# joybio/multiPrime

Measured on AMD Instinct MI355X. Metric: candidate x sequence coverage evals/s, higher is better.
Workload: dtype u32; 1 GPU; synthetic MSA 1048576 x 1000, k=18, v=1, 8 candidates/window, 950 windows, strict -c 2,3,-1 per GPU x 1 GPU(s) = BASELINE configs[3] itself (SURVEY 8d input 4; synthetic 1M x 1 kb; shape 1x1: row shards x window groups); rows_per_gpu=1048576, rows_total=1048576, cols=1000, k=18, variation=1, candidates_per_window=8, windows=950, parallelism=one GPU holds every row

## Files before the change

multiprime_amd/csrc/common.hpp:

```cpp
#pragma once

#include "../../include/mprime.h"

#include <hip/hip_runtime.h>

#include <algorithm>
#include <cstdarg>
#include <cstdio>
#include <cstdlib>
#include <cstring>
#include <numeric>
#include <utility>
#include <chrono>
#include <mutex>
#include <unordered_map>
#include <vector>

namespace mp {

constexpr int kBlock = 256;
constexpr uint32_t kEmpty = 0xFFFFFFFFu;
constexpr int kHashSlots = 4096;
constexpr int kHashLimit = 3584;
constexpr int kEvalCC = 8;
// ... 13 lines not shown

template <int NQ> struct NibT {
    uint64_t q[NQ];
    __device__ void clear() {
#pragma unroll
        for (int i = 0; i < NQ; i++) q[i] = 0;
    }
    __device__ uint32_t get(int j) const {
        const int wi = j >> 4;
        uint64_t w = q[0];
#pragma unroll
        for (int i = 1; i < NQ; i++) w = wi == i ? q[i] : w;
        return (uint32_t)(w >> (4 * (j & 15))) & 15u;
    }
    __device__ void set(int j, uint32_t v) {
        const int wi = j >> 4, sh = 4 * (j & 15);
#pragma unroll
        for (int i = 0; i < NQ; i++)
            if (wi == i) q[i] = (q[i] & ~(15ull << sh)) | ((uint64_t)v << sh);
    }
    __device__ void shift_up(int n) {
        const int s = 4 * n, ws = s >> 6, bs = s & 63;
        if (s == 0) return;
        uint64_t out[NQ];
#pragma unroll
        for (int i = 0; i < NQ; i++) {
            uint64_t a = 0, b = 0;
#pragma unroll
            for (int t = 0; t < NQ; t++) {
                if (t == i - ws) a = q[t];
                if (t == i - ws - 1) b = q[t];
            }
            out[i] = bs ? (a << bs) | (b >> (64 - bs)) : a;
        }
#pragma unroll
        for (int i = 0; i < NQ; i++) q[i] = out[i];
    }
};
typedef NibT<2> Nib;

struct EvalForm {
    enum Path : int8_t { None, RowsNarrow, RowsWide, Bits, BitsX } path = None;
    int8_t bits_shape = 0;
    int8_t chain_shape = -1;
    bool use_prog = false;
    int8_t x_shape = 0;
    int8_t row_variant = 0;
    int8_t row_vmode = 0;
};

}

struct Lap {
    bool on = getenv("MP_TRACE") != nullptr;
    hipStream_t st;
    std::chrono::steady_clock::time_point t = std::chrono::steady_clock::now();
    explicit Lap(hipStream_t s) : st(s) {}
    void operator()(const char *what) {
        if (!on) return;
        (void)hipStreamSynchronize(st);
        auto now = std::chrono::steady_clock::now();
        fprintf(stderr, "[mprime] %-28s %8.3f ms\n", what, std::chrono::duration<double, std::milli>(now - t).count());
        t = now;
    }
};

#ifndef MP_HIST_CM64
#define MP_HIST_CM64 2
#endif

struct mp_ctx {
    char err[512] = {0};
    int dev = 0;
    hipStream_t stream = nullptr;
    const void *rot_block = nullptr;
    size_t rot_cleared = 0;
    hipStream_t alt_stream = nullptr;
    int64_t bytes = 0;
    int n_rows = 0, n_pad = 0, n_chunks = 0, max_len = 0, ustride = 0;
    int reserve_cols = 0;
    uint32_t *planes = nullptr, *cum = nullptr, *ung = nullptr;
    unsigned long long *cols = nullptr;
    int32_t *lead = nullptr, *rstrip = nullptr, *rlen = nullptr;
    int p0 = 0, n_win = 0, k = 0, v = 0;
    bool wide = false;
    unsigned long long *excl = nullptr;
    int32_t *patch_count = nullptr, *patch_off = nullptr, *patch_cursor = nullptr;
    uint32_t *patch_words = nullptr;
    int32_t *patch_rows = nullptr;
    int n_patch = 0, max_patch = 0;
    bool p64 = false;
    mp::ExRec *ex = nullptr;
    int ex_cap = 0;
    int *ex_count = nullptr, *err_flag = nullptr;
    std::vector<mp::ExRec> ex_host;
    std::vector<mp::ExRec> ex_raw;
    hipStream_t ex_stream = nullptr;
    int ex_pending = 0;
    std::mutex ex_mu;
    int32_t *extra_off = nullptr;
    uint32_t *extra_words = nullptr;
    int n_extra = 0;
    std::vector<int32_t> h_patch_off, h_extra_off;
    uint32_t *pplanes = nullptr, *pvalid = nullptr;
    uint32_t *qplanes = nullptr, *qvalid = nullptr;
    bool qp_dirty = true;
    mp::PatchWin *pwin = nullptr;
    size_t pp_words = 0, pv_words = 0;
    int max_npw = 0;
    bool pp_dirty = true;
    unsigned long long *g_key = nullptr;
    uint32_t *g_cnt = nullptr, *g_min = nullptr;
    uint32_t *g_gap = nullptr;
    int32_t *g_idx = nullptr;
    int g_slots = 0;
    long long u_cap = 0, u_n = 0;
    uint32_t *u_b0 = nullptr, *u_b1 = nullptr, *u_g = nullptr;
    int32_t *u_count = nullptr, *u_first = nullptr, *labels = nullptr, *u_over = nullptr, *u_wcount = nullptr;
    int64_t *u_wbase = nullptr;
    unsigned long long *u_total = nullptr;
    std::vector<int64_t> h_wbase;
    std::vector<int32_t> h_wcount;
    double gate_threshold = 0;
    std::vector<uint8_t> h_wskip;
    uint8_t *dm_loss = nullptr;
    double *dm_dg = nullptr;
    std::vector<uint8_t> dm_loss_host;
    std::vector<double> dm_dg_host;
    unsigned long long *mask_f = nullptr, *mask_r = nullptr;
    size_t mask_words = 0;
    int n_masks = 0;
    int n_cand = 0, n_items = 0, n_padded = 0;
    mp::EvalItem *items = nullptr;
    uint4 *cand_n = nullptr;
    uint32_t *cand_symT = nullptr, *cand_diff = nullptr, *chain_events = nullptr;
    mp::ChainItem *chain_items = nullptr;
    void *x_items = nullptr;
    uint32_t *x_events = nullptr;
    int32_t *x_cand_out = nullptr;
    int x_n = 0, x_n_events = 0;
    int32_t *table_ids = nullptr;
    int n_chain = 0, n_table = 0, n_events = 0, max_steps = 0;
    std::vector<mp::ChainItem> h_chains;
    std::vector<uint32_t> h_events;
    std::vector<int32_t> h_cand_out;
    uint32_t *chain_prog = nullptr;
    size_t chain_prog_n = 0;
    mp::EvalForm form;
    mp::SlideBand *slide_bands = nullptr;
    uint32_t *slide_iters = nullptr, *slide_recs = nullptr;
    size_t slide_n_iters = 0;
    int slide_items = 0, slide_n_bands = 0, slide_max_items = 0, slide_ns = 0, slide_gw = 0;
    uint32_t slide_spos = 0, slide_fmask = 0, slide_rmask = 0, slide_fpos = 0, slide_rpos = 0;
    bool slide_fast = false;
    mp::ChainItem *chain_rest = nullptr;
    mp::ChainItem *chain_slid = nullptr;
    int n_rest = 0, rest_max_steps = 0;
    unsigned launch_seq = 0;
    int32_t *cand_out = nullptr;
    uint64_t sF = 0, sR = 0;
    unsigned long long *tmp_out = nullptr;
    int tmp_out_n = 0;
    struct PoolBlock { void *p; size_t bytes; hipEvent_t released; };
    std::vector<hipEvent_t> pool_events;
    std::unordered_map<void *, size_t> pool_live;
    std::vector<PoolBlock> pool;
    size_t pool_bytes = 0;
    long long pool_hits = 0, pool_misses = 0;
    int pool_on = -1;
    std::mutex pool_mu;
    unsigned long long *stats_buf = nullptr;
    size_t stats_buf_n = 0;
    std::vector<std::pair<hipEvent_t, hipEvent_t>> ev_busy, ev_free;
    double ev_ms = 0;
    std::vector<float> ev_samples, ev_last;
    int ev_n = 0;
    uint8_t *h_stage = nullptr;
    size_t h_stage_bytes = 0;
    bool h_stage_pinned = false;
    uint8_t *h_stats = nullptr;
    size_t h_stats_bytes = 0, stats_pending_f = 0, stats_pending_t = 0;
    bool h_stats_pinned = false;
    hipEvent_t stats_ev = nullptr;
    uint8_t *h_ring = nullptr;
    bool h_ring_pinned = false;
    hipEvent_t h_ring_ev[3] = {nullptr, nullptr, nullptr};
    uint8_t *sq_bytes = nullptr;
    int64_t *sq_roff = nullptr;
    unsigned long long *sq_code = nullptr, *sq_flag = nullptr;
    int64_t *sq_woff = nullptr;
    int32_t sq_n = 0;
    size_t sq_total = 0, sq_words = 0;
    std::vector<int64_t> sq_roff_host;
    int32_t *ot_out = nullptr;
    int64_t ot_n = 0;
    std::vector<uint8_t> ot_key;
    double ot_ms[4] = {0, 0, 0, 0};
    int64_t ot_counts[7] = {0, 0, 0, 0, 0, 0, 0};
    std::vector<int32_t> otc_out;
    std::vector<uint8_t> otc_key;
    uint8_t *an_code = nullptr;
    uint32_t *an_kmer = nullptr;
    int32_t *an_table = nullptr;
    int32_t *an_col = nullptr, *an_colinv = nullptr;
    int32_t an_n = 0, an_L = 0, an_slots = 0;
    int32_t an_par[6] = {0, 0, 0, 0, 0, 0};
    double an_ms[5] = {0, 0, 0, 0, 0};
    int64_t an_counts[3] = {0, 0, 0};
    int32_t an_both = 0;
    uint8_t *cl_code = nullptr;
    int64_t *cl_off = nullptr;
    int32_t cl_n = 0;
    size_t cl_total = 0;
    std::vector<int64_t> cl_off_host;
    double cl_ms[5] = {0, 0, 0, 0, 0};
    int64_t cl_counts[3] = {0, 0, 0};
    bool cl_rev = false;
    uint32_t *ani_sk = nullptr;
    int32_t *ani_sizes = nullptr;
    uint32_t *ani_tab = nullptr;
    int32_t ani_n = 0, ani_s = 0;
    uint32_t *ani_or = nullptr;
    bool ani_strands = false;
    double ani_ms[2] = {0, 0};
    int64_t ani_counts[2] = {0, 0};
    uint8_t *st_bytes = nullptr;
    int64_t *st_off = nullptr;
    int32_t st_n = 0;
    size_t st_total = 0;
    std::vector<int64_t> st_off_host;
    uint8_t *st_parity = nullptr;
    int32_t st_an = 0, st_stride = 0, st_width = 0;
    int32_t *st_d0 = nullptr, *st_end = nullptr, *st_meta = nullptr, *st_wfin = nullptr;
    uint8_t *st_arow = nullptr;
    uint16_t *st_runlen = nullptr, *st_qstart = nullptr;
    int32_t *st_ins = nullptr, *st_acol = nullptr;
    int32_t *st_colmap = nullptr;
    uint8_t *st_rows = nullptr;
    int32_t *st_colcnt = nullptr;
    double st_ms[8] = {0, 0, 0, 0, 0, 0, 0, 0};
    int64_t st_counts[6] = {0, 0, 0, 0, 0, 0};
    mp::DegeState *dege = nullptr;
    uint64_t *ont_keys = nullptr;
    int32_t *ont_q = nullptr;
    int32_t ont_n = 0, ont_max_len = 0;
    double ont_ms = 0;
    int64_t ont_counts[2] = {0, 0};
    mp::SetScreen *ss = nullptr;
    double ss_ms[4] = {0, 0, 0, 0};
    int64_t ss_counts[8] = {0, 0, 0, 0, 0, 0, 0, 0};
    void *comm = nullptr;
    int n_ranks = 0, rank = 0;
    uint8_t *comm_scratch = nullptr;
    size_t comm_scratch_n = 0;
};

namespace mp {


inline size_t wsz(const mp_ctx *c) { return c->wide ? 2 : 1; }

inline int fail(mp_ctx *c, int code, const char *fmt, ...) {
    va_list ap;
    va_start(ap, fmt);
    vsnprintf(c->err, sizeof c->err, fmt, ap);
    va_end(ap);
    return code;
}

#define HIPCK(c, call)                                                                                   \
    do {                                                                                                 \
        hipError_t e_ = (call);                                                                          \
        if (e_ != hipSuccess) return fail((c), MP_ERR_DEVICE, "%s: %s", #call, hipGetErrorString(e_));  \
    } while (0)

void *pool_take(mp_ctx *c, size_t bytes);
bool pool_give(mp_ctx *c, void *p, size_t bytes);
void pool_drain(mp_ctx *c);
void pool_drain_all();
void pool_register(mp_ctx *c, bool alive);
void pool_note(mp_ctx *c, void *p, size_t bytes);
size_t pool_forget(mp_ctx *c, void *p, size_t claimed);

template <typename T>
int dev_alloc(mp_ctx *c, T **p, size_t n) {
    *p = nullptr;
    if (n == 0) n = 1;
    if (void *q = pool_take(c, n * sizeof(T))) {
        *p = (T *)q;
        pool_note(c, q, n * sizeof(T));
        c->bytes += (int64_t)(n * sizeof(T));
        return MP_OK;
    }
    hipError_t e = hipMalloc((void **)p, n * sizeof(T));
    if (e != hipSuccess) {
        (void)hipGetLastError();
        pool_drain_all();
        e = hipMalloc((void **)p, n * sizeof(T));
    }
    if (e != hipSuccess) return fail(c, MP_ERR_NOMEM, "hipMalloc(%zu bytes): %s", n * sizeof(T), hipGetErrorString(e));
    pool_note(c, (void *)*p, n * sizeof(T));
    c->bytes += (int64_t)(n * sizeof(T));
    return MP_OK;
}

template <typename T>
// ... 38 lines not shown
```

multiprime_amd/csrc/evalslide.hip:

```cpp
#include "common.hpp"
#include "bitslice.hpp"
#include "slidecore.hpp"
#include "evalslide.hpp"
#include "chainbody.hpp"

using namespace mp;

namespace {

typedef unsigned int u32x4 __attribute__((ext_vector_type(4)));
typedef unsigned int u32x2 __attribute__((ext_vector_type(2)));

struct SlideKernArgs {
    SlideArgs A;
    const uint32_t *cols32;
    const uint32_t *excl32;
    int nw32;
    unsigned long long *out;
    int wc, wc_pad;
    int max_items;
    int n_slide_blocks;
    EvalChainArgs chain;
    unsigned long long *clear;
    uint32_t n_clear;
    int patch_words;
    unsigned long long *stamps;
};

template <int GW>
struct DevEnv {
    const SlideKernArgs &K;
    __amdgpu_buffer_rsrc_t rs_cols, rs_excl;
    int voff, lane;
    uint32_t row_bytes;
    bool live;
    uint32_t *ring;
    uint32_t *tab;
    uint32_t itv;
    uint32_t live_mask;

    __device__ __forceinline__ DevEnv(const SlideKernArgs &k) : K(k) {}
    __device__ __forceinline__ void progress(int quarter) const {
#ifndef SLIDE_NO_PRIO
        if (quarter <= 0) __builtin_amdgcn_s_setprio(3);
        else if (quarter == 1) __builtin_amdgcn_s_setprio(2);
        else if (quarter == 2) __builtin_amdgcn_s_setprio(1);
        else __builtin_amdgcn_s_setprio(0);
#endif
    }
    __device__ __forceinline__ void stamp(int i) const {
        if (K.stamps && threadIdx.x == 0) K.stamps[(size_t)blockIdx.x * 8 + i] = wall_clock64();
    }
    __device__ __forceinline__ SlideBand uband(int b) const {
        const SlideBand *p = K.A.bands + b;
        SlideBand r;
        r.w0 = __builtin_amdgcn_readfirstlane(p->w0); r.n_win = __builtin_amdgcn_readfirstlane(p->n_win);
        r.item0 = __builtin_amdgcn_readfirstlane(p->item0); r.n_items = __builtin_amdgcn_readfirstlane(p->n_items);
        r.iter0 = __builtin_amdgcn_readfirstlane(p->iter0); r.pad = 0;
        return r;
    }
    __device__ __forceinline__ void load_iters(int idx) { itv = K.A.iters[(size_t)idx + (size_t)lane]; }
    __device__ __forceinline__ uint32_t iter_word(int j) const { return (uint32_t)__builtin_amdgcn_readlane((int)itv, j); }
    typedef const uint32_t __attribute__((address_space(4))) * ConstWords;
    struct Rec { uint32_t w[8], sm_lo, sm_hi, flags; ConstWords p; };
    __device__ __forceinline__ Rec load_rec(int item) const {
        Rec r;
        r.p = (ConstWords)(K.A.recs + (size_t)__builtin_amdgcn_readfirstlane(item) * kSlideRec);
#pragma unroll
        for (int q = 0; q < 8; q++) r.w[q] = r.p[q];
        r.sm_lo = r.p[24]; r.sm_hi = r.p[25]; r.flags = r.p[28];
        return r;
    }
    __device__ __forceinline__ uint32_t rec_word(const Rec &r, int q) const {
        return q < 8 ? r.w[q] : (q == 24 ? r.sm_lo : (q == 25 ? r.sm_hi : (q == 28 ? r.flags : r.p[q])));
    }
    __device__ __forceinline__ uint32_t rec_word_dyn(const Rec &r, int q) const { return r.p[q]; }
    template <int AUX = 0>
    __device__ __forceinline__ void load(__amdgpu_buffer_rsrc_t rs, int soff, uint32_t (&d)[GW]) const {
        if constexpr (GW == 4) {
            const u32x4 v = __builtin_amdgcn_raw_buffer_load_b128(rs, voff, soff, AUX);
            d[0] = v.x; d[1] = v.y; d[2] = v.z; d[3] = v.w;
        } else if constexpr (GW == 2) {
            const u32x2 v = __builtin_amdgcn_raw_buffer_load_b64(rs, voff, soff, AUX);
            d[0] = v.x; d[1] = v.y;
        } else {
            d[0] = __builtin_amdgcn_raw_buffer_load_b32(rs, voff, soff, AUX);
        }
    }
#ifndef SLIDE_EXP_ONE_ROW
#define SLIDE_EXP_ONE_ROW 0
#endif
#ifndef SLIDE_COL_AUX
#define SLIDE_COL_AUX 2
#endif
#ifndef SLIDE_EVT_AUX
#define SLIDE_EVT_AUX 0
#endif
    __device__ __forceinline__ void fetch(uint32_t row_off, uint32_t (&d)[GW]) const {
        load<SLIDE_COL_AUX>(rs_cols, SLIDE_EXP_ONE_ROW == 1 || SLIDE_EXP_ONE_ROW == 3 ? 0 : (int)row_off, d);
    }
    __device__ __forceinline__ void fetch_event(uint32_t row_off, uint32_t (&d)[GW]) const {
        load<SLIDE_EVT_AUX>(rs_cols, SLIDE_EXP_ONE_ROW == 1 || SLIDE_EXP_ONE_ROW == 2 ? 0 : (int)row_off, d);
    }
    __device__ __forceinline__ void valid_of(uint32_t row_off, uint32_t (&v)[GW]) const {
        load(rs_excl, (int)row_off, v);
#pragma unroll
        for (int i = 0; i < GW; i++) v[i] = bop<kSlAndNot>(live_mask, v[i], 0u);
    }
    __device__ __forceinline__ void ring_put(uint32_t *p, const uint32_t (&v)[GW]) const {
        if constexpr (GW == 4) *reinterpret_cast<u32x4 *>(p) = u32x4{v[0], v[1], v[2], v[3]};
        else if constexpr (GW == 2) *reinterpret_cast<u32x2 *>(p) = u32x2{v[0], v[1]};
        else p[0] = v[0];
    }
    __device__ __forceinline__ void ring_get(const uint32_t *p, uint32_t (&v)[GW]) const {
        if constexpr (GW == 4) { const u32x4 t = *reinterpret_cast<const u32x4 *>(p); v[0] = t.x; v[1] = t.y; v[2] = t.z; v[3] = t.w; }
        else if constexpr (GW == 2) { const u32x2 t = *reinterpret_cast<const u32x2 *>(p); v[0] = t.x; v[1] = t.y; }
        else v[0] = p[0];
    }
    __device__ __forceinline__ void ring_zero(int k) {
        uint32_t z[GW];
#pragma unroll
        for (int i = 0; i < GW; i++) z[i] = 0u;
        for (int s = 0; s < k; s++) ring_put(ring + s * (64 * GW), z);
    }
    __device__ __forceinline__ uint32_t ring_step() const { return 64u * GW * (uint32_t)sizeof(uint32_t); }
    __device__ __forceinline__ uint32_t *ring_at(uint32_t off) const { return reinterpret_cast<uint32_t *>(reinterpret_cast<char *>(ring) + off); }
    __device__ __forceinline__ void ring_write(uint32_t off, const uint32_t (&in)[GW]) { ring_put(ring_at(off), in); }
    __device__ __forceinline__ void ring_read(uint32_t off, uint32_t (&o)[GW]) const { ring_get(ring_at(off), o); }
    __device__ __forceinline__ void commit(int idx, const uint32_t (&accPF)[8], const uint32_t (&accR)[4]) {
        uint32_t x0 = accPF[0], x1 = accPF[1], x2 = accPF[2], x3 = accPF[3], x4 = accPF[4], x5 = accPF[5], x6 = accPF[6], x7 = accPF[7];
        uint32_t x8 = accR[0], x9 = accR[1], x10 = accR[2], x11 = accR[3];
        asm volatile(
            "s_nop 1\n\t"
            "v_add_u32_dpp %0, %0, %0 row_ror:4 row_mask:0xf bank_mask:0x5\n\t"
            "v_add_u32_dpp %2, %2, %2 row_ror:4 row_mask:0xf bank_mask:0x5\n\t"
            "v_add_u32_dpp %4, %4, %4 row_ror:4 row_mask:0xf bank_mask:0x5\n\t"
            "v_add_u32_dpp %6, %6, %6 row_ror:4 row_mask:0xf bank_mask:0x5\n\t"
            "v_add_u32_dpp %8, %8, %8 row_ror:4 row_mask:0xf bank_mask:0x5\n\t"
            "v_add_u32_dpp %10, %10, %10 row_ror:4 row_mask:0xf bank_mask:0x5\n\t"
            "v_add_u32_dpp %0, %1, %1 row_ror:4 row_mask:0xf bank_mask:0xa\n\t"
            "v_add_u32_dpp %2, %3, %3 row_ror:4 row_mask:0xf bank_mask:0xa\n\t"
            "v_add_u32_dpp %4, %5, %5 row_ror:4 row_mask:0xf bank_mask:0xa\n\t"
            "v_add_u32_dpp %6, %7, %7 row_ror:4 row_mask:0xf bank_mask:0xa\n\t"
            "v_add_u32_dpp %8, %9, %9 row_ror:4 row_mask:0xf bank_mask:0xa\n\t"
            "v_add_u32_dpp %10, %11, %11 row_ror:4 row_mask:0xf bank_mask:0xa\n\t"
            "v_add_u32_dpp %0, %0, %0 row_ror:8 row_mask:0xf bank_mask:0x3\n\t"
            "v_add_u32_dpp %4, %4, %4 row_ror:8 row_mask:0xf bank_mask:0x3\n\t"
            "v_add_u32_dpp %8, %8, %8 row_ror:8 row_mask:0xf bank_mask:0x3\n\t"
            "v_add_u32_dpp %0, %2, %2 row_ror:8 row_mask:0xf bank_mask:0xc\n\t"
            "v_add_u32_dpp %4, %6, %6 row_ror:8 row_mask:0xf bank_mask:0xc\n\t"
            "v_add_u32_dpp %8, %10, %10 row_ror:8 row_mask:0xf bank_mask:0xc\n\t"
            "v_add_u32_dpp %0, %0, %0 quad_perm:[1,0,3,2] row_mask:0xf bank_mask:0xf\n\t"
            "v_add_u32_dpp %4, %4, %4 quad_perm:[1,0,3,2] row_mask:0xf bank_mask:0xf\n\t"
            "v_add_u32_dpp %8, %8, %8 quad_perm:[1,0,3,2] row_mask:0xf bank_mask:0xf\n\t"
            "v_add_u32_dpp %0, %0, %0 quad_perm:[2,3,0,1] row_mask:0xf bank_mask:0xf\n\t"
            "v_add_u32_dpp %4, %4, %4 quad_perm:[2,3,0,1] row_mask:0xf bank_mask:0xf\n\t"
            "v_add_u32_dpp %8, %8, %8 quad_perm:[2,3,0,1] row_mask:0xf bank_mask:0xf\n\t"
            "s_nop 1"
            : "+v"(x0), "+v"(x1), "+v"(x2), "+v"(x3), "+v"(x4), "+v"(x5), "+v"(x6), "+v"(x7), "+v"(x8), "+v"(x9), "+v"(x10), "+v"(x11));
        typedef unsigned int u32pair __attribute__((ext_vector_type(2)));
        const u32pair s01 = __builtin_amdgcn_permlane16_swap(x0, x4, false, false);
        const uint32_t a = s01.x + s01.y;
        const u32pair s22 = __builtin_amdgcn_permlane16_swap(x8, x8, false, false);
        const uint32_t b = s22.x + s22.y;
        const u32pair h = __builtin_amdgcn_permlane32_swap(a, b, false, false);
        const uint32_t tot = h.x + h.y;
        if (lane < 48 && (lane & 3) == 0) atomicAdd(&tab[idx * 12 + (lane >> 4) * 4 + ((lane >> 2) & 3)], tot);
    }
};

#ifndef SLIDE_MIN_WAVES
#define SLIDE_MIN_WAVES 1
#endif
template <int LV, int GW, bool FAST>
__global__ __launch_bounds__(kBlock, GW == 4 ? 1 : SLIDE_MIN_WAVES) void eval_slide_kernel(const SlideKernArgs K) {
    extern __shared__ __align__(16) uint32_t lds[];
    clear_counters(K.clear, K.n_clear, blockIdx.x, gridDim.x);
    if (K.stamps && threadIdx.x == 0) K.stamps[(size_t)blockIdx.x * 8] = wall_clock64();
    if ((int)blockIdx.x >= K.n_slide_blocks) {
        const unsigned pb = blockIdx.x - (unsigned)K.n_slide_blocks, wv = threadIdx.x >> 6;
#ifndef SLIDE_PATCH_PRIO
#define SLIDE_PATCH_PRIO 3
#endif
        __builtin_amdgcn_s_setprio(SLIDE_PATCH_PRIO);
        if (K.patch_words == 1) {
            const bool negative = (int)pb >= K.chain.patch.n_blocks;
            const unsigned unit = (pb - (negative ? (unsigned)K.chain.patch.n_blocks : 0u)) * (kBlock / 64) + wv;
            eval_patch_wave<LV>(K.chain, lds + wv * 12, lds + 64 + wv * (64 * kPatchEvents), unit, negative);
        } else {
            uint32_t(&s_part)[kBlock / 64][12] = *reinterpret_cast<uint32_t(*)[kBlock / 64][12]>(lds);
            eval_chain_block<LV, 8, 4>(K.chain, s_part, pb);
        }
        if (K.stamps && threadIdx.x == 0) K.stamps[(size_t)blockIdx.x * 8 + 7] = wall_clock64();
        return;
    }
    const int slice = (int)(blockIdx.x % (unsigned)K.wc_pad), band = (int)(blockIdx.x / (unsigned)K.wc_pad);
    if (slice >= K.wc) return;
    const int wv = (int)(threadIdx.x >> 6), lane = (int)(threadIdx.x & 63);
    const int ring_words = K.A.k * 64 * GW;
    uint32_t *tab = lds + (kBlock / 64) * ring_words;
    DevEnv<GW> env(K);
    env.lane = lane;
    env.ring = lds + wv * ring_words + lane * GW;
    env.tab = tab;
    env.itv = 0u;
    const int word0 = (slice * kBlock + (int)threadIdx.x) * GW;
    env.live = word0 < K.nw32;
    env.voff = env.live ? word0 * 4 : 0x7FFFFF00;
    env.live_mask = env.live ? 0xFFFFFFFFu : 0u;
    env.row_bytes = (uint32_t)K.nw32 * 4u;
    env.rs_cols = __builtin_amdgcn_make_buffer_rsrc(const_cast<uint32_t *>(K.cols32), 0, 0x7FFFFF00, 0x00020000);
    env.rs_excl = __builtin_amdgcn_make_buffer_rsrc(const_cast<uint32_t *>(K.excl32), 0, 0x7FFFFF00, 0x00020000);
    const SlideBand bd = env.uband(band);
    for (int i = (int)threadIdx.x; i < bd.n_items * 12; i += kBlock) tab[i] = 0u;
    __syncthreads();
    env.stamp(1);
    const bool wave_live = (slice * kBlock + wv * 64) * GW < K.nw32;
    if (wave_live) slide_band<LV, GW, true, false, FAST>(env, K.A, band);
    env.stamp(4);
    __syncthreads();
    env.stamp(5);
    int live_waves = 0;
    for (int w = 0; w < kBlock / 64; w++) live_waves += (slice * kBlock + w * 64) * GW < K.nw32 ? 1 : 0;
    const uint32_t rows = (uint32_t)live_waves * 64u * 32u * GW;
    const int n_entries = bd.n_items * 24;
    for (int i0 = (int)threadIdx.x; i0 < n_entries; i0 += 4 * kBlock) {
        int oc[4];
        uint32_t map[4];
#pragma unroll
        for (int u = 0; u < 4; u++) {
            const int i = i0 + u * kBlock, ic = i < n_entries ? i : (int)threadIdx.x;
            const uint32_t *rec = K.A.recs + (size_t)(bd.item0 + ic / 24) * kSlideRec;
            oc[u] = (int)rec[8 + (ic % 24) / 3];
            map[u] = rec[26];
        }
#pragma unroll
        for (int u = 0; u < 4; u++) {
            const int i = i0 + u * kBlock;
            if (i >= n_entries || oc[u] < 0) continue;
            const int item = i / 24, r = i % 24, t = r / 3, kind = r % 3;
            const int slot = (int)((map[u] >> (4 * t)) & 15u);
            const uint32_t *row = tab + item * 12;
            const uint32_t out1 = row[slot] & 0xFFFFu, outF = row[slot] >> 16, outR = (row[8 + (slot >> 1)] >> (16 * (slot & 1))) & 0xFFFFu;
            const uint32_t val = kind == 0 ? rows - out1 : out1 - (kind == 1 ? outF : outR);
            if (val) atomicAdd(&K.out[(size_t)oc[u] * 3 + kind], (unsigned long long)val);
        }
    }
    env.stamp(6);
}

typedef void (*SlideFn)(const SlideKernArgs);

}

namespace mp {

void free_slide(mp_ctx *c) {
    dev_free(c, &c->slide_bands, (size_t)c->slide_n_bands);
    dev_free(c, &c->slide_iters, c->slide_n_iters);
    dev_free(c, &c->slide_recs, (size_t)c->slide_items * kSlideRec);
    dev_free(c, &c->chain_rest, (size_t)c->n_rest);
    dev_free(c, &c->chain_slid, (size_t)c->slide_items);
    c->slide_items = c->slide_n_bands = c->slide_max_items = 0;
    c->slide_n_iters = 0;
    c->n_rest = c->rest_max_steps = 0;
}

int upload_eval_slide(mp_ctx *c, const std::vector<ChainItem> &chains, const std::vector<uint32_t> &events, const std::vector<int32_t> &cand_out) {
    free_slide(c);
    const char *se = getenv("MP_EVAL_SLIDE");
    if (chains.empty() || c->v > 3 || c->k <= c->v || (se ? atoi(se) != 1 : c->n_pad <= 262144)) return MP_OK;
    const int nw32 = c->n_pad / 32, n_cols = c->n_chunks * 32;
    if (((unsigned long long)n_cols * 4ull + 1ull) * (unsigned long long)nw32 * 4ull >= 0x7FFFFFFFull) return MP_OK;
    if ((unsigned long long)c->n_win * (unsigned long long)nw32 * 4ull >= 0x7FFFFFFFull) return MP_OK;
    int gw = 2;
    if (const char *e = getenv("MP_SLIDE_GW")) { const int g = atoi(e); if (g == 1 || g == 2 || g == 4) gw = g; }
    const int wc = (nw32 + kBlock * gw - 1) / (kBlock * gw), wc_pad = wc >= 8 ? (wc + 7) / 8 * 8 : wc;
    const int span = chains.back().win - chains.front().win + 1;
    std::vector<SlideChainIn> in(chains.size());
    for (size_t i = 0; i < chains.size(); i++) {
        const ChainItem &ch = chains[i];
        in[i] = SlideChainIn{ch.win, ch.cand0, ch.n_steps, ch.ev0, ch.n_ev, {ch.sym[0], ch.sym[1], ch.sym[2], ch.sym[3]}};
    }
    const size_t ring_bytes = (size_t)(kBlock / 64) * ((size_t)c->k * 64 * gw) * sizeof(uint32_t), lds_cu = 160 * 1024;
    int resident = (int)std::min<size_t>(4, std::max<size_t>(1, lds_cu / (ring_bytes + 1024)));
    if (gw == 4) resident = 1;
    SlidePlan P;
    for (;; resident--) {
        const int per_round = std::max(1, 256 * resident / std::max(1, wc_pad));
        int band = (span + per_round - 1) / per_round;
        for (int r = 2; band > 96; r++) band = (span + per_round * r - 1) / (per_round * r);
        band = std::max(8, band);
        if (const char *e = getenv("MP_SLIDE_BAND")) band = std::max(1, atoi(e));
        if (!build_slide_plan(in, events, cand_out, c->k, (uint32_t)c->sF, (uint32_t)c->sR, c->p0, n_cols, band, (uint32_t)nw32 * 4u, true, P)) return MP_OK;
        const size_t need = ring_bytes + (size_t)P.max_items_band * 12 * sizeof(uint32_t);
        if (resident <= 1 || need * (size_t)resident <= lds_cu) break;
    }
    P.iters.resize(P.iters.size() + 64, 0u);
    int rc;
    if ((rc = dev_alloc(c, &c->slide_bands, P.bands.size()))) return rc;
    c->slide_n_bands = (int)P.bands.size();
    if ((rc = dev_alloc(c, &c->slide_iters, P.iters.size()))) return rc;
    c->slide_n_iters = P.iters.size();
    c->slide_items = (int)P.item_of.size();
    if ((rc = dev_alloc(c, &c->slide_recs, P.recs.size()))) return rc;
    HIPCK(c, hipMemcpy(c->slide_bands, P.bands.data(), sizeof(SlideBand) * P.bands.size(), hipMemcpyHostToDevice));
    HIPCK(c, hipMemcpy(c->slide_iters, P.iters.data(), sizeof(uint32_t) * P.iters.size(), hipMemcpyHostToDevice));
    HIPCK(c, hipMemcpy(c->slide_recs, P.recs.data(), sizeof(uint32_t) * P.recs.size(), hipMemcpyHostToDevice));
    c->slide_max_items = P.max_items_band;
    c->slide_ns = P.ns; c->slide_spos = P.spos; c->slide_fmask = P.fmask; c->slide_rmask = P.rmask;
    c->slide_fast = slide_strict_lists(c->k, (uint32_t)c->sF, (uint32_t)c->sR, c->slide_fpos, c->slide_rpos);
    if (const char *e = getenv("MP_SLIDE_STRICT")) { if (atoi(e) == 0) c->slide_fast = false; }
    c->slide_gw = gw;
    {
        std::vector<ChainItem> slid;
        for (int32_t i : P.item_of) slid.push_back(chains[(size_t)i]);
        if ((rc = dev_alloc(c, &c->chain_slid, slid.size()))) return rc;
        HIPCK(c, hipMemcpy(c->chain_slid, slid.data(), sizeof(ChainItem) * slid.size(), hipMemcpyHostToDevice));
    }
    if (!P.rest.empty()) {
        std::vector<ChainItem> rest;
        for (int32_t i : P.rest) { rest.push_back(chains[(size_t)i]); c->rest_max_steps = std::max(c->rest_max_steps, (int)chains[(size_t)i].n_steps); }
        if ((rc = dev_alloc(c, &c->chain_rest, rest.size()))) return rc;
        c->n_rest = (int)rest.size();
        HIPCK(c, hipMemcpy(c->chain_rest, rest.data(), sizeof(ChainItem) * rest.size(), hipMemcpyHostToDevice));
    }
    return MP_OK;
}

int launch_eval_slide(mp_ctx *c, unsigned long long *device_out, const EvalChainArgs *patch, int patch_blocks, int patch_words,
                      unsigned long long *clear, uint32_t n_clear) {
#define SLIDE_ROW(LV, F) {eval_slide_kernel<LV, 1, F>, eval_slide_kernel<LV, 2, F>, eval_slide_kernel<LV, 4, F>}
    static const SlideFn fn[2][4][3] = {{SLIDE_ROW(1, false), SLIDE_ROW(2, false), SLIDE_ROW(3, false), SLIDE_ROW(4, false)},
                                        {SLIDE_ROW(1, true), SLIDE_ROW(2, true), SLIDE_ROW(3, true), SLIDE_ROW(4, true)}};
#undef SLIDE_ROW
    const int gw = c->slide_gw, gi = gw == 4 ? 2 : gw - 1;
    const int nw32 = c->n_pad / 32;
    SlideKernArgs K;
    K.A = SlideArgs{c->slide_bands, c->slide_iters, c->slide_recs, c->k, c->p0, c->slide_ns, c->slide_spos, c->slide_fmask, c->slide_rmask,
                    (uint32_t)nw32 * 4u, c->slide_fpos, c->slide_rpos, 0u, 0u};
    if (c->slide_fast) slide_strict_distinct(c->slide_fpos, c->slide_rpos, K.A.dpos, K.A.dshape);
    K.cols32 = reinterpret_cast<const uint32_t *>(c->cols);
    K.excl32 = reinterpret_cast<const uint32_t *>(c->excl);
    K.nw32 = nw32;
    K.out = device_out;
    K.wc = (nw32 + kBlock * gw - 1) / (kBlock * gw);
    K.wc_pad = K.wc >= 8 ? (K.wc + 7) / 8 * 8 : K.wc;
    K.max_items = c->slide_max_items;
    K.n_slide_blocks = c->slide_n_bands * K.wc_pad;
    if (patch) K.chain = *patch;
    else { memset(&K.chain, 0, sizeof K.chain); patch_blocks = 0; }
    K.chain.clear = nullptr; K.chain.n_clear = 0;
    K.clear = clear; K.n_clear = n_clear;
    K.patch_words = patch_words;
    K.stamps = nullptr;
    const char *stamp_file = getenv("MP_EXPERIMENT_STAMPS");
    const size_t n_stamp = ((size_t)K.n_slide_blocks + (size_t)patch_blocks) * 8;
    if (stamp_file) {
        HIPCK(c, hipMalloc(&K.stamps, n_stamp * sizeof(unsigned long long)));
        HIPCK(c, hipMemsetAsync(K.stamps, 0, n_stamp * sizeof(unsigned long long), c->stream));
    }
    size_t lds = ((size_t)(kBlock / 64) * ((size_t)c->k * 64 * gw) + (size_t)c->slide_max_items * 12) * sizeof(uint32_t);
    if (patch_blocks) lds = std::max(lds, (size_t)(64 + (kBlock / 64) * 64 * kPatchEvents) * sizeof(uint32_t));
    if (lds > 160 * 1024) return fail(c, MP_ERR_ARG, "sliding evaluation: a band needs %zu bytes of LDS", lds);
    SlideFn f = fn[c->slide_fast ? 1 : 0][c->v][gi];
    if (lds > 48 * 1024) HIPCK(c, hipFuncSetAttribute(reinterpret_cast<const void *>(f), hipFuncAttributeMaxDynamicSharedMemorySize, (int)lds));
    hipLaunchKernelGGL(f, dim3((unsigned)K.n_slide_blocks + (unsigned)patch_blocks), dim3(kBlock), lds, c->stream, K);
    HIPCK(c, hipGetLastError());
    if (stamp_file) {
        std::vector<unsigned long long> h(n_stamp + 2);
        HIPCK(c, hipStreamSynchronize(c->stream));
        HIPCK(c, hipMemcpy(h.data() + 2, K.stamps, n_stamp * sizeof(unsigned long long), hipMemcpyDeviceToHost));
        HIPCK(c, hipFree(K.stamps));
        h[0] = (unsigned long long)K.n_slide_blocks; h[1] = (unsigned long long)patch_blocks;
        if (FILE *fo = fopen(stamp_file, "wb")) { fwrite(h.data(), sizeof(unsigned long long), h.size(), fo); fclose(fo); }
    }
    return MP_OK;
}

}
```

multiprime_amd/csrc/slidecore.hpp:

```cpp
#pragma once

#include <cstdint>

#include "slideplan.hpp"

#if defined(__HIPCC__)
#define SLIDE_HD __host__ __device__ __forceinline__
#else
#define SLIDE_HD inline
#endif

#ifndef SLIDE_UNLIKELY
#define SLIDE_UNLIKELY(x) __builtin_expect(!!(x), 0)
#endif

namespace mp {

template <int LUT>
SLIDE_HD uint32_t bop(uint32_t a, uint32_t b, uint32_t c) {
#if defined(__HIP_DEVICE_COMPILE__)
    return __builtin_amdgcn_bitop3_b32(a, b, c, LUT);
#else
    uint32_t r = 0;
    if (LUT & 0x01) r |= ~a & ~b & ~c;
// ... 302 lines not shown
    }
}

template <int N, int GW, class Env>
SLIDE_HD void slide_warm_chunk(Env &env, SlideCount (&cnt)[GW], uint32_t &cur, int j) {
    uint32_t w[N][GW];
#pragma unroll
    for (int u = 0; u < N; u++) env.fetch(env.iter_word(2 * (j + u)), w[u]);
#pragma unroll
    for (int u = 0; u < N; u++) {
        uint32_t bn[GW];
#pragma unroll
        for (int i = 0; i < GW; i++) {
            bn[i] = ~w[u][i];
            slide_updown(cnt[i], bn[i], bn[i]);
        }
        env.ring_write(cur, bn);
        cur += env.ring_step();
    }
}

template <int LV, int GW, bool ONLY_SIMPLE, bool USE_VALID, bool FAST = false, class Env>
SLIDE_HD void slide_band(Env &env, const SlideArgs &A, int band_index) {
    static_assert(LV >= 1 && LV <= 4 && GW >= 1 && GW <= 4, "counter levels / words per lane");
    static_assert(!FAST || ONLY_SIMPLE, "FAST strict counts: simple items only");
    const SlideBand bd = env.uband(band_index);
    const int k = A.k;
    SlideCount cnt[GW];
#pragma unroll
    for (int i = 0; i < GW; i++) cnt[i] = SlideCount{0u, 0u, 0u, 0u, 0u};
    env.ring_zero(k);
    const uint32_t ring_step = env.ring_step(), ring_end = (uint32_t)k * ring_step;
    uint32_t cur = 0u;
    const int n_iter = bd.n_win + k - 1;
    const int last_item = bd.item0 + bd.n_items - 1;
    typename Env::Rec rec0 = env.load_rec(bd.item0), rec1 = env.load_rec(bd.item0 + 1 <= last_item ? bd.item0 + 1 : last_item);
    SlideFetch<GW> F0, F1;
    slide_request<GW, USE_VALID>(env, rec0, F0);
    int done = 0;
    env.load_iters(bd.iter0);
    env.stamp(2);
    int j0 = 0;
    {
        const int n_warm = k - 1 < n_iter ? k - 1 : n_iter;
        while (n_warm - j0 >= 16) { slide_warm_chunk<16, GW>(env, cnt, cur, j0); j0 += 16; }
        if (n_warm - j0 >= 8) { slide_warm_chunk<8, GW>(env, cnt, cur, j0); j0 += 8; }
        if (n_warm - j0 >= 4) { slide_warm_chunk<4, GW>(env, cnt, cur, j0); j0 += 4; }
        if (n_warm - j0 >= 2) { slide_warm_chunk<2, GW>(env, cnt, cur, j0); j0 += 2; }
    }
    env.stamp(3);
    uint32_t bA[GW], bB[GW];
    env.fetch(env.iter_word(2 * j0), bA);
    env.fetch(env.iter_word(n_iter > j0 + 1 ? 2 * j0 + 2 : 2 * j0), bB);

    auto item = [&](typename Env::Rec &rec_cur, typename Env::Rec &rec_other, const SlideFetch<GW> &F_cur, SlideFetch<GW> &F_other,
                    const uint32_t (&sv)[kSlideStrict][GW]) __attribute__((always_inline)) {
        const int after = bd.item0 + done + 2;
        const typename Env::Rec rec = rec_cur;
        rec_cur = env.load_rec(after <= last_item ? after : last_item);
        slide_request<GW, USE_VALID>(env, rec_other, F_other);
        const uint32_t hdr = env.rec_word(rec, 0);
        uint32_t accPF[8], accR[4];
        if (ONLY_SIMPLE || (hdr & kSlSimple)) slide_item<LV, GW, true, USE_VALID, ONLY_SIMPLE, FAST>(env, A, rec, hdr, cnt, sv, F_cur, accPF, accR);
        else slide_item<LV, GW, false, USE_VALID, false, false>(env, A, rec, hdr, cnt, sv, F_cur, accPF, accR);
        env.commit(done, accPF, accR);
        done++;
    };
#ifndef SLIDE_PRIO_MIN_WIN
#define SLIDE_PRIO_MIN_WIN 32
#endif
    const int quarter_len = bd.n_win < SLIDE_PRIO_MIN_WIN ? 1 << 20 : ((bd.n_win + 3) / 4 > 2 ? (bd.n_win + 3) / 4 : 2);
    auto run = [&](auto shape) __attribute__((always_inline)) {
        typedef decltype(shape) Shape;
        constexpr int NS = Shape::ND;
        uint32_t so[NS > 0 ? NS : 1], sm[NS > 0 ? NS : 1];
#pragma unroll
        for (int q = 0; q < NS; q++) {
            uint32_t pos, present = 1u;
            if (!FAST) pos = (A.spos >> (5 * q)) & 31u;
            else if (!Shape::MASKED) pos = (A.dpos >> (5 * q)) & 31u;
            else {
                const uint32_t list = q < 3 ? A.fpos : A.rpos;
                const int qq = q < 3 ? q : q - 3;
                present = qq < (int)(list >> 15) ? 1u : 0u;
                pos = present ? (list >> (5 * qq)) & 31u : 0u;
            }
            so[q] = (((uint32_t)j0 + pos) % (uint32_t)k) * ring_step;
            sm[q] = present ? 0xFFFFFFFFu : 0u;
        }
        auto iteration = [&](uint32_t (&b)[GW], uint32_t (&bo)[GW], uint32_t (&bo_next)[GW], int j) __attribute__((always_inline)) {
            const uint32_t it1 = env.iter_word(2 * j + 1);
            uint32_t bn[GW];
#pragma unroll
            for (int i = 0; i < GW; i++) bn[i] = ~b[i];
            env.fetch(env.iter_word(2 * j + 4), b);
#pragma unroll
            for (int i = 0; i < GW; i++) slide_updown(cnt[i], bn[i] ^ bo[i], bn[i]);
            env.ring_write(cur, bn);
            cur += ring_step;
            if (cur == ring_end) cur = 0u;
            env.ring_read(cur, bo_next);
#pragma unroll
            for (int q = 0; q < NS; q++) {
                so[q] += ring_step;
                if (so[q] == ring_end) so[q] = 0u;
            }
            const int n_items = (int)(it1 >> 24);
            if (n_items == 0) return;
            uint32_t sv[kSlideStrict][GW];
            if (FAST) {
                uint32_t d[NS > 0 ? NS : 1][GW];
#pragma unroll
                for (int q = 0; q < NS; q++) {
                    env.ring_read(so[q], d[q]);
                    if (Shape::MASKED) {
#pragma unroll
                        for (int i = 0; i < GW; i++) d[q][i] &= sm[q];
                    }
                }
                constexpr int NF = Shape::NB + Shape::NFO, NR = Shape::NB + Shape::NRO;
                static_assert(NF <= 3 && NR <= 3, "at most three strict positions per side");
#pragma unroll
                for (int i = 0; i < GW; i++) {
                    uint32_t f[3] = {0u, 0u, 0u}, r[3] = {0u, 0u, 0u};
#pragma unroll
                    for (int q = 0; q < NF; q++) f[q] = d[q][i];
#pragma unroll
                    for (int q = 0; q < NR; q++) r[q] = d[q < Shape::NB ? q : q + Shape::NFO][i];
                    sv[0][i] = NF == 3 ? bop<kSlXor3>(f[0], f[1], f[2]) : (f[0] ^ f[1]);
                    sv[1][i] = NF == 3 ? bop<kSlMaj>(f[0], f[1], f[2]) : (f[0] & f[1]);
                    sv[2][i] = NR == 3 ? bop<kSlXor3>(r[0], r[1], r[2]) : (r[0] ^ r[1]);
                    sv[3][i] = NR == 3 ? bop<kSlMaj>(r[0], r[1], r[2]) : (r[0] & r[1]);
                }
            }
#pragma unroll
            for (int q = 0; q < kSlideStrict; q++) {
                if (FAST) break;
                if (q < NS) {
                    env.ring_read(so[q], sv[q]);
                } else {
#pragma unroll
                    for (int i = 0; i < GW; i++) sv[q][i] = 0u;
                }
            }
            int ii = 0;
            if (done & 1) { item(rec1, rec0, F1, F0, sv); ii = 1; }
#pragma unroll 1
            for (; ii + 1 < n_items; ii += 2) {
                item(rec0, rec1, F0, F1, sv);
                item(rec1, rec0, F1, F0, sv);
            }
            if (ii < n_items) item(rec0, rec1, F0, F1, sv);
        };
        int quarter = 0, next_quarter = k - 1 + quarter_len;
        env.progress(0);
        uint32_t boA[GW], boB[GW];
        env.ring_read(cur, boA);
#pragma unroll 1
        for (int base = 0; base < n_iter; base += 30) {
            if (base) env.load_iters(bd.iter0 + 2 * base);
            const int n_here = n_iter - base < 30 ? n_iter - base : 30;
            int j = base ? 0 : j0;
#pragma unroll 1
            for (; j + 1 < n_here; j += 2) {
                if (base + j >= next_quarter) { env.progress(++quarter); next_quarter += quarter_len; }
                iteration(bA, boA, boB, j);
                iteration(bB, boB, boA, j + 1);
            }
            if (j < n_here) iteration(bA, boA, boB, j);
        }
    };
    if constexpr (!FAST) {
        if (A.ns > 4) run(SlideShape<0, 3, 3, false>());
        else run(SlideShape<0, 2, 2, false>());
    } else {
        switch (A.dshape) {
            case kSlShapeDefault: run(SlideShape<1, 1, 2, false>()); break;
            case slide_shape_code(0, 0, 0): run(SlideShape<0, 0, 0, false>()); break;
            case slide_shape_code(1, 0, 0): run(SlideShape<1, 0, 0, false>()); break;
            case slide_shape_code(0, 1, 1): run(SlideShape<0, 1, 1, false>()); break;
            case slide_shape_code(0, 2, 2): run(SlideShape<0, 2, 2, false>()); break;
            case slide_shape_code(0, 3, 3): run(SlideShape<0, 3, 3, false>()); break;
            default: run(SlideShape<0, 3, 3, true>()); break;
        }
    }
    env.progress(3);
}

}
```

multiprime_amd/csrc/slideplan.hpp:

```cpp
#pragma once

#include <algorithm>
#include <cstdint>
#include <cstring>
#include <vector>

namespace mp {

constexpr int kSlideRec = 32;
constexpr int kSlideKept = 7;
constexpr int kSlideExtra = 8;
constexpr int kSlideStrict = 6;
constexpr uint32_t kSlPresent = 1u << 7, kSlSub = 1u << 8, kSlStrictF = 1u << 9, kSlStrictR = 1u << 10;
constexpr uint32_t kSlSimple = 1u << 16;

struct SlideChainIn {
    int32_t win, cand0, n_steps, ev0, n_ev;
    uint32_t sym[4];
};

struct SlideBand { int32_t w0, n_win, item0, n_items, iter0, pad; };

struct SlidePlan {
    std::vector<uint8_t> slides;
    std::vector<int32_t> rest;
    std::vector<int32_t> item_of;
    std::vector<SlideBand> bands;
    std::vector<uint32_t> iters;
    std::vector<uint32_t> recs;
    std::vector<uint8_t> ref;
    int k = 0, ns = 0, max_items_band = 0;
    uint32_t spos = 0, fmask = 0, rmask = 0;
};

inline bool slide_record(const SlideChainIn &ch, const std::vector<uint32_t> &events, const std::vector<int32_t> &cand_out, int k, uint32_t sF,
                         uint32_t sR, int p0, const std::vector<uint8_t> &ref, const int (&slot_of_pos)[32], uint32_t row_scale,
                         uint32_t zero_row, uint32_t *rec) {
    auto sym = [&](int j) { return (ch.sym[j >> 3] >> (4 * (j & 7))) & 15u; };
    for (int q = 0; q < kSlideRec; q++) rec[q] = 0u;
    if (ch.n_steps < 1 || ch.n_steps > 8) return false;
    for (int m = 0; m < 8; m++) rec[8 + m] = 0xFFFFFFFFu;
    for (int q = 1; q <= kSlideKept; q++) rec[q] = zero_row * row_scale;
    const uint32_t row0 = (uint32_t)(p0 + ch.win) * 4u;
    int cur = 0, e = 0;
    rec[8] = (uint32_t)cand_out[(size_t)ch.cand0];
    bool lost_seen[32 * 4] = {false};
    bool simple = true;
    for (int t = 1; t < ch.n_steps; t++) {
        while (e < ch.n_ev && (int)(events[(size_t)ch.ev0 + (size_t)e] >> 16) == t) {
            const uint32_t ev = events[(size_t)ch.ev0 + (size_t)e];
            const int j = (int)(ev & 255u), base = __builtin_ctz((ev >> 8) & 15u);
            if (++cur > kSlideKept) return false;
            rec[cur] = (row0 + (uint32_t)(j * 4 + base)) * row_scale;
            if ((sF >> j) & 1u) rec[28] |= 1u << cur;
            if ((sR >> j) & 1u) rec[28] |= 1u << (8 + cur);
            if (base != ref[(size_t)(p0 + ch.win + j)]) {
                rec[28] |= 1u << (16 + cur);
                if (slot_of_pos[j] >= 0) rec[24 + slot_of_pos[j] / 4] |= (1u << cur) << (8 * (slot_of_pos[j] & 3));
            } else {
                simple = false;
            }
            lost_seen[j * 4 + base] = true;
            e++;
        }
        rec[8 + t] = (uint32_t)cand_out[(size_t)ch.cand0 + (size_t)t];
        rec[26] |= (uint32_t)cur << (4 * t);
    }
    if (e != ch.n_ev) return false;
    int nx = 0;
    for (int j = 0; j < k; j++) {
        const uint32_t sy = sym(j);
        const int r = ref[(size_t)(p0 + ch.win + j)];
        for (int b = 0; b < 4; b++) {
            const bool in_s0 = sy >> b & 1u;
            const bool sub = in_s0 && b != r && !lost_seen[j * 4 + b], add = !in_s0 && b == r;
            if (!sub && !add) continue;
            if (slot_of_pos[j] >= 0 || nx == kSlideExtra) return false;
            rec[16 + nx++] = (uint32_t)(j * 4 + b) | kSlPresent | (sub ? kSlSub : 0u);
        }
    }
    rec[0] = (uint32_t)(cur + 1) | ((uint32_t)nx << 8) | (simple ? kSlSimple : 0u);
    rec[27] = (uint32_t)ch.win;
    rec[29] = (uint32_t)ch.win * row_scale;
    rec[30] = row0 * row_scale;
    return true;
}

inline bool build_slide_plan(const std::vector<SlideChainIn> &chains, const std::vector<uint32_t> &events, const std::vector<int32_t> &cand_out,
                             int k, uint32_t sF, uint32_t sR, int p0, int n_cols, int band_windows, uint32_t row_scale, bool simple_only,
                             SlidePlan &P) {
    P = SlidePlan();
    P.k = k;
    if (k < 2 || k > 31 || chains.empty()) return false;
    const uint32_t kmask = (1u << k) - 1u;
    int slot_of_pos[32];
    for (int j = 0; j < 32; j++) slot_of_pos[j] = -1;
    for (int j = 0; j < k; j++)
        if (((sF | sR) & kmask) >> j & 1u) {
            if (P.ns == kSlideStrict) return false;
            slot_of_pos[j] = P.ns;
            P.spos |= (uint32_t)j << (5 * P.ns);
            if ((sF >> j) & 1u) P.fmask |= 1u << P.ns;
            if ((sR >> j) & 1u) P.rmask |= 1u << P.ns;
            P.ns++;
        }
    auto sym = [](const SlideChainIn &ch, int j) { return (ch.sym[j >> 3] >> (4 * (j & 7))) & 15u; };
    std::vector<int32_t> votes((size_t)n_cols * 4, 0);
    for (const SlideChainIn &ch : chains) {
        if (ch.win < 0 || p0 + ch.win + k > n_cols) return false;
        for (int j = 0; j < k; j++)
            for (int b = 0; b < 4; b++)
                if (sym(ch, j) >> b & 1u) votes[(size_t)(p0 + ch.win + j) * 4 + b]++;
    }
    P.ref.assign((size_t)n_cols, 0);
    for (int c = 0; c < n_cols; c++) {
        int best = 0;
        for (int b = 1; b < 4; b++)
            if (votes[(size_t)c * 4 + b] > votes[(size_t)c * 4 + best]) best = b;
        P.ref[(size_t)c] = (uint8_t)best;
    }
    P.slides.assign(chains.size(), 0);
    std::vector<uint32_t> rec((size_t)kSlideRec);
    for (size_t i = 0; i < chains.size(); i++) {
        if (i && chains[i].win < chains[i - 1].win) return false;
        if (slide_record(chains[i], events, cand_out, k, sF, sR, p0, P.ref, slot_of_pos, row_scale, (uint32_t)n_cols * 4u, rec.data()) &&
            (!simple_only || ((rec[0] & kSlSimple) && ((rec[0] >> 8) & 15u) == 0))) {
            P.slides[i] = 1;
            P.item_of.push_back((int32_t)i);
            P.recs.insert(P.recs.end(), rec.begin(), rec.end());
        } else {
            P.rest.push_back((int32_t)i);
        }
    }
    if (P.item_of.empty()) return false;
    const int B = std::max(1, band_windows);
    const size_t n = P.item_of.size();
    auto win_of = [&](size_t pi) { return chains[(size_t)P.item_of[pi]].win; };
    size_t i = 0;
    while (i < n) {
        SlideBand bd{win_of(i), 1, (int32_t)i, 0, (int32_t)P.iters.size(), 0};
        size_t j = i;
        int last = win_of(i);
        while (j < n) {
            const int w = win_of(j);
            if (w - bd.w0 + 1 > B || w - last > k - 1) break;
            last = w;
            j++;
        }
        bd.n_win = last - bd.w0 + 1;
        bd.n_items = (int32_t)(j - i);
        P.max_items_band = std::max(P.max_items_band, (int)bd.n_items);
        size_t it = i;
        for (int t = -(k - 1); t < bd.n_win; t++) {
            const int col = p0 + bd.w0 + t + k - 1;
            uint32_t first = (uint32_t)(it - i), cnt = 0;
            if (t >= 0)
                while (it < j && win_of(it) == bd.w0 + t) { it++; cnt++; }
            if (cnt > 255) return false;
            P.iters.push_back(((uint32_t)col * 4u + P.ref[(size_t)col]) * row_scale);
            P.iters.push_back(first | (cnt << 24));
        }
        P.bands.push_back(bd);
        i = j;
    }
    return true;
}

}
```

Before: 67550 billion evals/s.

## Pick slide group width automatically from residency and make priority ladder configurable

Moves the sliding-plan residency and band sizing into slideplan helpers and adds an automatic choice of group width. Large inputs with low two-word residency now use one word per lane with higher occupancy launch bounds. It also adds a runtime-selectable priority scheme (none, ladder, low-entry) and a configurable patch-block priority. The aim is more resident waves per CU on large row counts, in exchange for more sliding blocks and different register pressure.

```diff
diff --git a/multiprime_amd/csrc/common.hpp b/multiprime_amd/csrc/common.hpp
--- a/multiprime_amd/csrc/common.hpp
+++ b/multiprime_amd/csrc/common.hpp
@@ -189,6 +189,7 @@
     size_t slide_n_iters = 0;
     int slide_items = 0, slide_n_bands = 0, slide_max_items = 0, slide_ns = 0, slide_gw = 0;
     uint32_t slide_spos = 0, slide_fmask = 0, slide_rmask = 0, slide_fpos = 0, slide_rpos = 0;
+    int slide_prio = 0;
     bool slide_fast = false;
     mp::ChainItem *chain_rest = nullptr;
     mp::ChainItem *chain_slid = nullptr;
diff --git a/multiprime_amd/csrc/evalslide.hip b/multiprime_amd/csrc/evalslide.hip
--- a/multiprime_amd/csrc/evalslide.hip
+++ b/multiprime_amd/csrc/evalslide.hip
@@ -24,6 +24,7 @@
     unsigned long long *clear;
     uint32_t n_clear;
     int patch_words;
+    int prio;
     unsigned long long *stamps;
 };
 
@@ -42,12 +43,15 @@
     __device__ __forceinline__ DevEnv(const SlideKernArgs &k) : K(k) {}
     __device__ __forceinline__ void progress(int quarter) const {
 #ifndef SLIDE_NO_PRIO
-        if (quarter <= 0) __builtin_amdgcn_s_setprio(3);
+        if ((K.prio & 3) == kSlidePrioNone) return;
+        if (quarter < 0) __builtin_amdgcn_s_setprio(0);
+        else if (quarter == 0) __builtin_amdgcn_s_setprio(3);
         else if (quarter == 1) __builtin_amdgcn_s_setprio(2);
         else if (quarter == 2) __builtin_amdgcn_s_setprio(1);
         else __builtin_amdgcn_s_setprio(0);
 #endif
     }
+    __device__ __forceinline__ bool low_entry() const { return (K.prio & 3) == kSlidePrioLow; }
     __device__ __forceinline__ void stamp(int i) const {
         if (K.stamps && threadIdx.x == 0) K.stamps[(size_t)blockIdx.x * 8 + i] = wall_clock64();
     }
@@ -169,20 +173,24 @@
     }
 };
 
+static_assert(kBlock == 64 * kSlideWaves, "a sliding workgroup is one wave per SIMD");
+static_assert(slide_reg_resident(2) == 4 && slide_reg_resident(1) == 5 && slide_reg_resident(4) == 1, "launch bounds below");
 #ifndef SLIDE_MIN_WAVES
 #define SLIDE_MIN_WAVES 1
 #endif
 template <int LV, int GW, bool FAST>
-__global__ __launch_bounds__(kBlock, GW == 4 ? 1 : SLIDE_MIN_WAVES) void eval_slide_kernel(const SlideKernArgs K) {
+__global__ __launch_bounds__(kBlock, GW == 2 ? SLIDE_MIN_WAVES : slide_reg_resident(GW)) void eval_slide_kernel(const SlideKernArgs K) {
     extern __shared__ __align__(16) uint32_t lds[];
     clear_counters(K.clear, K.n_clear, blockIdx.x, gridDim.x);
     if (K.stamps && threadIdx.x == 0) K.stamps[(size_t)blockIdx.x * 8] = wall_clock64();
     if ((int)blockIdx.x >= K.n_slide_blocks) {
         const unsigned pb = blockIdx.x - (unsigned)K.n_slide_blocks, wv = threadIdx.x >> 6;
-#ifndef SLIDE_PATCH_PRIO
-#define SLIDE_PATCH_PRIO 3
-#endif
-        __builtin_amdgcn_s_setprio(SLIDE_PATCH_PRIO);
+        switch ((K.prio >> 4) & 3) {
+            case 3: __builtin_amdgcn_s_setprio(3); break;
+            case 2: __builtin_amdgcn_s_setprio(2); break;
+            case 1: __builtin_amdgcn_s_setprio(1); break;
+            default: break;
+        }
         if (K.patch_words == 1) {
             const bool negative = (int)pb >= K.chain.patch.n_blocks;
             const unsigned unit = (pb - (negative ? (unsigned)K.chain.patch.n_blocks : 0u)) * (kBlock / 64) + wv;
@@ -273,28 +281,22 @@
     const int nw32 = c->n_pad / 32, n_cols = c->n_chunks * 32;
     if (((unsigned long long)n_cols * 4ull + 1ull) * (unsigned long long)nw32 * 4ull >= 0x7FFFFFFFull) return MP_OK;
     if ((unsigned long long)c->n_win * (unsigned long long)nw32 * 4ull >= 0x7FFFFFFFull) return MP_OK;
-    int gw = 2;
+    int gw = 0;
     if (const char *e = getenv("MP_SLIDE_GW")) { const int g = atoi(e); if (g == 1 || g == 2 || g == 4) gw = g; }
-    const int wc = (nw32 + kBlock * gw - 1) / (kBlock * gw), wc_pad = wc >= 8 ? (wc + 7) / 8 * 8 : wc;
-    const int span = chains.back().win - chains.front().win + 1;
     std::vector<SlideChainIn> in(chains.size());
     for (size_t i = 0; i < chains.size(); i++) {
         const ChainItem &ch = chains[i];
         in[i] = SlideChainIn{ch.win, ch.cand0, ch.n_steps, ch.ev0, ch.n_ev, {ch.sym[0], ch.sym[1], ch.sym[2], ch.sym[3]}};
     }
-    const size_t ring_bytes = (size_t)(kBlock / 64) * ((size_t)c->k * 64 * gw) * sizeof(uint32_t), lds_cu = 160 * 1024;
-    int resident = (int)std::min<size_t>(4, std::max<size_t>(1, lds_cu / (ring_bytes + 1024)));
-    if (gw == 4) resident = 1;
+    int resident = 0, cap = 0, band_override = 0;
+    if (const char *e = getenv("MP_SLIDE_RESIDENT")) cap = std::max(0, atoi(e));
+    if (const char *e = getenv("MP_SLIDE_BAND")) band_override = std::max(1, atoi(e));
     SlidePlan P;
-    for (;; resident--) {
-        const int per_round = std::max(1, 256 * resident / std::max(1, wc_pad));
-        int band = (span + per_round - 1) / per_round;
-        for (int r = 2; band > 96; r++) band = (span + per_round * r - 1) / (per_round * r);
-        band = std::max(8, band);
-        if (const char *e = getenv("MP_SLIDE_BAND")) band = std::max(1, atoi(e));
-        if (!build_slide_plan(in, events, cand_out, c->k, (uint32_t)c->sF, (uint32_t)c->sR, c->p0, n_cols, band, (uint32_t)nw32 * 4u, true, P)) return MP_OK;
-        const size_t need = ring_bytes + (size_t)P.max_items_band * 12 * sizeof(uint32_t);
-        if (resident <= 1 || need * (size_t)resident <= lds_cu) break;
+    if (gw) {
+        if (!build_slide_plan_resident(in, events, cand_out, c->k, (uint32_t)c->sF, (uint32_t)c->sR, c->p0, n_cols, nw32, gw, cap, band_override, P, resident))
+            return MP_OK;
+    } else if (!(gw = build_slide_plan_auto(in, events, cand_out, c->k, (uint32_t)c->sF, (uint32_t)c->sR, c->p0, n_cols, nw32, cap, band_override, P, resident))) {
+        return MP_OK;
     }
     P.iters.resize(P.iters.size() + 64, 0u);
     int rc;
@@ -312,6 +314,10 @@
     c->slide_fast = slide_strict_lists(c->k, (uint32_t)c->sF, (uint32_t)c->sR, c->slide_fpos, c->slide_rpos);
     if (const char *e = getenv("MP_SLIDE_STRICT")) { if (atoi(e) == 0) c->slide_fast = false; }
     c->slide_gw = gw;
+    int ladder = kSlidePrioLadder, patch_prio = 3;
+    if (const char *e = getenv("MP_SLIDE_PRIO")) ladder = std::min(2, std::max(0, atoi(e)));
+    if (const char *e = getenv("MP_SLIDE_PATCH_PRIO")) patch_prio = std::min(3, std::max(0, atoi(e)));
+    c->slide_prio = ladder | (patch_prio << 4);
     {
         std::vector<ChainItem> slid;
         for (int32_t i : P.item_of) slid.push_back(chains[(size_t)i]);
@@ -353,6 +359,7 @@
     K.chain.clear = nullptr; K.chain.n_clear = 0;
     K.clear = clear; K.n_clear = n_clear;
     K.patch_words = patch_words;
+    K.prio = c->slide_prio;
     K.stamps = nullptr;
     const char *stamp_file = getenv("MP_EXPERIMENT_STAMPS");
     const size_t n_stamp = ((size_t)K.n_slide_blocks + (size_t)patch_blocks) * 8;
@@ -360,7 +367,7 @@
         HIPCK(c, hipMalloc(&K.stamps, n_stamp * sizeof(unsigned long long)));
         HIPCK(c, hipMemsetAsync(K.stamps, 0, n_stamp * sizeof(unsigned long long), c->stream));
     }
-    size_t lds = ((size_t)(kBlock / 64) * ((size_t)c->k * 64 * gw) + (size_t)c->slide_max_items * 12) * sizeof(uint32_t);
+    size_t lds = slide_lds_need(gw, c->k, c->slide_max_items);
     if (patch_blocks) lds = std::max(lds, (size_t)(64 + (kBlock / 64) * 64 * kPatchEvents) * sizeof(uint32_t));
     if (lds > 160 * 1024) return fail(c, MP_ERR_ARG, "sliding evaluation: a band needs %zu bytes of LDS", lds);
     SlideFn f = fn[c->slide_fast ? 1 : 0][c->v][gi];
diff --git a/multiprime_amd/csrc/slidecore.hpp b/multiprime_amd/csrc/slidecore.hpp
--- a/multiprime_amd/csrc/slidecore.hpp
+++ b/multiprime_amd/csrc/slidecore.hpp
@@ -478,8 +478,9 @@
             }
             if (ii < n_items) item(rec0, rec1, F0, F1, sv);
         };
-        int quarter = 0, next_quarter = k - 1 + quarter_len;
-        env.progress(0);
+        const bool low = env.low_entry();
+        int quarter = low ? -1 : 0, next_quarter = low ? k - 1 : k - 1 + quarter_len;
+        env.progress(quarter);
         uint32_t boA[GW], boB[GW];
         env.ring_read(cur, boA);
 #pragma unroll 1
diff --git a/multiprime_amd/csrc/slideplan.hpp b/multiprime_amd/csrc/slideplan.hpp
--- a/multiprime_amd/csrc/slideplan.hpp
+++ b/multiprime_amd/csrc/slideplan.hpp
@@ -20,6 +20,36 @@
 };
 
 struct SlideBand { int32_t w0, n_win, item0, n_items, iter0, pad; };
+
+constexpr int kSlideWaves = 4;
+constexpr size_t kSlideLdsCu = 160 * 1024;
+constexpr int kSlideCus = 256;
+constexpr int slide_reg_resident(int gw) { return gw == 1 ? 5 : (gw == 2 ? 4 : 1); }
+inline size_t slide_ring_bytes(int gw, int k) { return (size_t)kSlideWaves * ((size_t)k * 64 * (size_t)gw) * sizeof(uint32_t); }
+inline size_t slide_lds_need(int gw, int k, int max_items_band) { return slide_ring_bytes(gw, k) + (size_t)max_items_band * 12 * sizeof(uint32_t); }
+inline int slide_resident_start(int gw, int k, int cap = 0) {
+    int r = (int)std::min<size_t>((size_t)slide_reg_resident(gw), std::max<size_t>(1, kSlideLdsCu / (slide_ring_bytes(gw, k) + 1024)));
+    if (cap > 0) r = std::min(r, cap);
+    return std::max(1, r);
+}
+inline bool slide_fits(int gw, int k, int max_items_band, int resident) {
+    return resident <= 1 || slide_lds_need(gw, k, max_items_band) * (size_t)resident <= kSlideLdsCu;
+}
+inline int slide_band_len(int span, int wc_pad, int resident) {
+    const int per_round = std::max(1, kSlideCus * resident / std::max(1, wc_pad));
+    int band = (span + per_round - 1) / per_round;
+    for (int r = 2; band > 96; r++) band = (span + per_round * r - 1) / (per_round * r);
+    return std::max(8, band);
+}
+inline int slide_slices(int nw32, int gw, int *padded = nullptr) {
+    const int wc = (nw32 + 64 * kSlideWaves * gw - 1) / (64 * kSlideWaves * gw);
+    if (padded) *padded = wc >= 8 ? (wc + 7) / 8 * 8 : wc;
+    return wc;
+}
+
+constexpr int kSlidePrioNone = 0, kSlidePrioLadder = 1, kSlidePrioLow = 2;
+constexpr int kSlideFirstPassRows = 262144;
+inline int slide_default_gw(int n_pad, int resident_two_words) { return n_pad > kSlideFirstPassRows && resident_two_words < 3 ? 1 : 2; }
 
 struct SlidePlan {
     std::vector<uint8_t> slides;
@@ -166,4 +196,25 @@
     return true;
 }
 
-}
+inline bool build_slide_plan_resident(const std::vector<SlideChainIn> &chains, const std::vector<uint32_t> &events, const std::vector<int32_t> &cand_out,
+                                      int k, uint32_t sF, uint32_t sR, int p0, int n_cols, int nw32, int gw, int cap, int band_override, SlidePlan &P,
+                                      int &resident) {
+    if (chains.empty()) return false;
+    const int span = chains.back().win - chains.front().win + 1;
+    int wc_pad;
+    slide_slices(nw32, gw, &wc_pad);
+    for (resident = slide_resident_start(gw, k, cap);; resident--) {
+        const int band = band_override > 0 ? band_override : slide_band_len(span, wc_pad, resident);
+        if (!build_slide_plan(chains, events, cand_out, k, sF, sR, p0, n_cols, band, (uint32_t)nw32 * 4u, true, P)) return false;
+        if (slide_fits(gw, k, P.max_items_band, resident)) return true;
+    }
+}
+
+inline int build_slide_plan_auto(const std::vector<SlideChainIn> &chains, const std::vector<uint32_t> &events, const std::vector<int32_t> &cand_out, int k,
+                                 uint32_t sF, uint32_t sR, int p0, int n_cols, int nw32, int cap, int band_override, SlidePlan &P, int &resident) {
+    if (!build_slide_plan_resident(chains, events, cand_out, k, sF, sR, p0, n_cols, nw32, 2, cap, band_override, P, resident)) return 0;
+    if (slide_default_gw(nw32 * 32, resident) == 2) return 2;
+    return build_slide_plan_resident(chains, events, cand_out, k, sF, sR, p0, n_cols, nw32, 1, cap, band_override, P, resident) ? 1 : 0;
+}
+
+}
```

After: 67040 billion evals/s. Within noise of the previous version (-0.7%).
